# avi22bhattacharya/ThinkDiff-mlre

Hardware: AMD Instinct MI355X
Metric: images/sec (1024², 28 steps) ThinkDiff-CLIP FLUX.1 at 1/2/4/8 MI355X (higher is better)
Workload: dtype bf16

## Files before the change

### thinkdiff-mlre_amd/csrc/elementwise.hip

```cpp
#include "td_common.h"
#include "td_kernels.h"
#include "qk_rope_math.h"
#include "../../include/thinkdiff_hip.h"

namespace {

__device__ __forceinline__ void unpack8(const u32x4_t v, float (&f)[8]) {
#pragma unroll
  for (int i = 0; i < 4; ++i) {
    f[2 * i] = bf_lo(v[i]);
    f[2 * i + 1] = bf_hi(v[i]);
  }
}
__device__ __forceinline__ u32x4_t pack8(const float (&f)[8]) {
  u32x4_t v;
#pragma unroll
  for (int i = 0; i < 4; ++i) v[i] = pack_bf2(f[2 * i], f[2 * i + 1]);
  return v;
}

}

__device__ __forceinline__ u32x2_t pack8_fp8(const float (&x)[8], float inv) {
  int lo = 0, hi = 0;
  lo = __builtin_amdgcn_cvt_pk_fp8_f32(x[0] * inv, x[1] * inv, lo, false);
  lo = __builtin_amdgcn_cvt_pk_fp8_f32(x[2] * inv, x[3] * inv, lo, true);
  hi = __builtin_amdgcn_cvt_pk_fp8_f32(x[4] * inv, x[5] * inv, hi, false);
  hi = __builtin_amdgcn_cvt_pk_fp8_f32(x[6] * inv, x[7] * inv, hi, true);
  return u32x2_t{(unsigned)lo, (unsigned)hi};
}
__device__ __forceinline__ u32x2_t pack8_i8(const float (&x)[8], float inv) {
  unsigned w[2];
#pragma unroll
  for (int h = 0; h < 2; ++h) {
    const unsigned b0 = (unsigned)__float2int_rn(x[4 * h] * inv) & 0xffu, b1 = (unsigned)__float2int_rn(x[4 * h + 1] * inv) & 0xffu;
    const unsigned b2 = (unsigned)__float2int_rn(x[4 * h + 2] * inv) & 0xffu, b3 = (unsigned)__float2int_rn(x[4 * h + 3] * inv) & 0xffu;
    w[h] = b0 | (b1 << 8) | (b2 << 16) | (b3 << 24);
  }
  return u32x2_t{w[0], w[1]};
}
__device__ __forceinline__ u32x2_t pack8_q(const float (&x)[8], float inv, bool int8) { return int8 ? pack8_i8(x, inv) : pack8_fp8(x, inv); }

template <int NCH>
__global__ __launch_bounds__(256) void td_norm_rows_kernel(const TdNormParams p) {
  const int lane = threadIdx.x & 63;
  const int row = blockIdx.x * 4 + (threadIdx.x >> 6);
  if (row >= p.rows) return;
  const bf16_t* xr = p.x + (size_t)row * p.ldx;
  int ext_s0 = -1, ext_s1 = -1;
  {
    const int* ext0 = row >= p.split ? p.extB : p.extA;
    if (p.q && ext0 && lane * 2 < p.ext_n) { ext_s0 = ext0[lane * 2]; ext_s1 = ext0[lane * 2 + 1]; }
  }
  float v[NCH][8];
  float sum = 0.f;
#pragma unroll
  for (int c = 0; c < NCH; ++c) {
    unpack8(*(const u32x4_t*)(xr + c * 512 + lane * 8), v[c]);
#pragma unroll
    for (int i = 0; i < 8; ++i) sum += v[c][i];
  }
  constexpr float inv_d = 1.0f / (NCH * 512);
  float mean = 0.f;
  if (!p.rms) mean = wave_sum(sum) * inv_d;
  float sq = 0.f;
#pragma unroll
  for (int c = 0; c < NCH; ++c)
#pragma unroll
    for (int i = 0; i < 8; ++i) {
      v[c][i] -= mean;
      sq += v[c][i] * v[c][i];
    }
  const float rstd = rsqrtf(wave_sum(sq) * inv_d + p.eps);

  const bool partB = row >= p.split;
  const bf16_t* shift = partB ? p.shiftB : p.shiftA;
  const bf16_t* scale = partB ? p.scaleB : p.scaleA;
  bf16_t* yr = p.y + (size_t)row * p.ldy;
  float amax = 0.f;
#pragma unroll
  for (int c = 0; c < NCH; ++c) {
    const int col = c * 512 + lane * 8;
    float y[8];
    const bool keep_f32 = p.rms == 2;
#pragma unroll
    for (int i = 0; i < 8; ++i) y[i] = keep_f32 ? v[c][i] * rstd : rbf(v[c][i] * rstd);
    if (p.w) {
      float w[8];
      unpack8(*(const u32x4_t*)(p.w + col), w);
#pragma unroll
      for (int i = 0; i < 8; ++i) y[i] = keep_f32 ? y[i] * w[i] : rbf(y[i] * w[i]);
    }
    if (scale) {
      float sc[8], sh[8];
      unpack8(*(const u32x4_t*)(scale + col), sc);
      unpack8(*(const u32x4_t*)(shift + col), sh);
#pragma unroll
      for (int i = 0; i < 8; ++i) y[i] = rbf(rbf(y[i] * rbf(1.0f + sc[i])) + sh[i]);
    }
    if (p.q) {
      float sm[8] = {1.f, 1.f, 1.f, 1.f, 1.f, 1.f, 1.f, 1.f};
      const bf16_t* smooth = partB ? p.smoothB : p.smoothA;
      if (smooth) unpack8(*(const u32x4_t*)(smooth + col), sm);
#pragma unroll
      for (int i = 0; i < 8; ++i) {
        v[c][i] = rbf(y[i]) * sm[i];
        amax = fmaxf(amax, fabsf(v[c][i]));
      }
    } else {
      *(u32x4_t*)(yr + col) = pack8(y);
    }
  }
  if (p.q) {
    amax = wave_max(amax);
    const float s = amax > 0.f ? amax * (p.q_int8 ? 1.0f / 127.0f : 1.0f / 448.0f) : 1.0f;
    const float inv = 1.0f / s;
    if (lane == 0) p.q_scale[row] = s;
    uint8_t* qr = p.q + (size_t)row * p.ldq;
    const int* ext = partB ? p.extB : p.extA;
    __shared__ __attribute__((aligned(8))) uint8_t qrow[4][NCH * 512];
#pragma unroll
    for (int c = 0; c < NCH; ++c) {
      const u32x2_t b = pack8_q(v[c], inv, p.q_int8 != 0);
      *(u32x2_t*)(qr + c * 512 + lane * 8) = b;
      if (ext) *(u32x2_t*)(&qrow[threadIdx.x >> 6][c * 512 + lane * 8]) = b;
    }
    if (ext) {
      for (int e = lane * 2; e < p.ext_n; e += 128) {
        const int s0 = e < 128 ? ext_s0 : ext[e], s1 = e < 128 ? ext_s1 : ext[e + 1];
        const unsigned b0 = s0 >= 0 ? qrow[threadIdx.x >> 6][s0] : 0u, b1 = s1 >= 0 ? qrow[threadIdx.x >> 6][s1] : 0u;
        *(unsigned short*)(qr + NCH * 512 + e) = (unsigned short)(b0 | (b1 << 8));
      }
    }
  }
}

int td_norm_rows_launch(const TdNormParams& p, hipStream_t stream) {
  TD_CHECK_ARG(p.rows > 0 && p.D > 0, "td_norm_rows: empty problem");
  TD_CHECK_ARG(p.D % 512 == 0 && p.D <= 4096, "td_norm_rows: D=%d must be a multiple of 512, <= 4096", p.D);
  TD_CHECK_ARG(p.ldx % 8 == 0 && p.ldy % 8 == 0, "td_norm_rows: row strides must be multiples of 8");
  TD_CHECK_ARG((p.scaleA == nullptr) == (p.shiftA == nullptr), "td_norm_rows: shift and scale come together");
  if (p.q) TD_CHECK_ARG(p.q_scale && p.ldq % 8 == 0 && (uintptr_t)p.q % 8 == 0, "td_norm_rows: fp8 output needs a scale array and 8-byte aligned rows");
  if (p.extA || p.extB) TD_CHECK_ARG(p.q && p.q_int8 && p.extA && p.extB && p.ext_n > 0 && p.ext_n % 2 == 0 && p.ldq >= p.D + p.ext_n,
                                     "td_norm_rows: replicated channels need the int8 output form, both tables and rows of D + ext_n bytes");
  TD_GRID_1D(nblk, (long long)((p.rows + 3) / 4) * 256, 256, "td_norm_rows");
  const dim3 grid(nblk), block(256);
  switch (p.D / 512) {
#define TD_CASE(n) case n: hipLaunchKernelGGL(td_norm_rows_kernel<n>, grid, block, 0, stream, p); break;
    TD_CASE(1) TD_CASE(2) TD_CASE(3) TD_CASE(4) TD_CASE(5) TD_CASE(6) TD_CASE(7) TD_CASE(8)
#undef TD_CASE
  }
  TD_CHECK_LAUNCH();
  return 0;
}

__global__ __launch_bounds__(256) void td_qk_norm_rope_kernel(const TdQkRopeParams p) {
  const int row = blockIdx.x;
  const int l16 = threadIdx.x & 15;
  const int unit0 = threadIdx.x >> 4;
  const int nunits = p.Hq + p.Hk;
  bf16_t* base = p.qkv + (size_t)row * p.ld;
  const bool partB = row >= p.split;
  const bf16_t* wq = partB ? p.wqB : p.wqA;
  const bf16_t* wk = partB ? p.wkB : p.wkA;

  float cs[8], sn[8];
  {
    const float* cr = p.cos + (size_t)row * 128;
    const float* sr = p.sin + (size_t)row * 128;
    const int d0 = l16 * 8;
#pragma unroll
    for (int i = 0; i < 8; i += 4) {
      const f32x4_t c4 = *(const f32x4_t*)(cr + d0 + i);
      const f32x4_t s4 = *(const f32x4_t*)(sr + d0 + i);
#pragma unroll
      for (int j = 0; j < 4; ++j) {
        cs[i + j] = c4[j];
        sn[i + j] = s4[j];
      }
    }
  }

  for (int u = unit0; u < nunits; u += 16) {
    const bool is_k = u >= p.Hq;
    bf16_t* hp = base + (is_k ? p.k_col + (u - p.Hq) * 128 : p.q_col + u * 128) + l16 * 8;
    float x[8];
    unpack8(*(const u32x4_t*)hp, x);
    const bf16_t* w = is_k ? wk : wq;
    if (w) {
      float sq = qk_sumsq8(x);
#pragma unroll
      for (int o = 8; o > 0; o >>= 1) sq += __shfl_xor(sq, o, 16);
      float wv[8];
      unpack8(*(const u32x4_t*)(w + l16 * 8), wv);
      qk_norm8(x, qk_rstd(sq, p.eps), wv);
    }
    float y[8];
    if (p.rotate_half) {
#pragma unroll
      for (int i = 0; i < 8; ++i) {
        const float other = __shfl_xor(x[i], 8, 16);
        const float rot = (l16 < 8) ? -other : other;
        y[i] = p.rotate_half == 2 ? qk_rope_half_rbf(x[i], other, l16 < 8, cs[i], sn[i]) : x[i] * cs[i] + rot * sn[i];
      }
    } else {
      qk_rope_pairs8(x, cs, sn, y);
    }
    if (!is_k && p.q_premul != 1.0f) {
#pragma unroll
      for (int i = 0; i < 8; ++i) y[i] *= p.q_premul;
    }
    *(u32x4_t*)hp = pack8(y);
  }
}

int td_qk_norm_rope_launch(const TdQkRopeParams& p, hipStream_t stream) {
  TD_CHECK_ARG(p.rows > 0 && p.Hq > 0 && p.Hk >= 0, "td_qk_norm_rope: empty problem");
  TD_CHECK_ARG(p.ld % 8 == 0 && p.q_col % 8 == 0 && p.k_col % 8 == 0, "td_qk_norm_rope: columns must be 16-byte aligned");
  TD_CHECK_ARG(p.rotate_half >= 0 && p.rotate_half <= 2, "td_qk_norm_rope: rotate_half=%d is not a rotation mode (0, 1 or 2)", p.rotate_half);
  TD_GRID_1D(nblk, (long long)p.rows * 256, 256, "td_qk_norm_rope");
  hipLaunchKernelGGL(td_qk_norm_rope_kernel, dim3(nblk), dim3(256), 0, stream, p);
  TD_CHECK_LAUNCH();
  return 0;
}

__global__ void td_flux_rope_table_kernel(const float* ids, int S, int d0, int d1, int d2, double theta, float* cosT, float* sinT) {
  const int idx = blockIdx.x * blockDim.x + threadIdx.x;
  const int half = (d0 + d1 + d2) / 2;
  if (idx >= S * half) return;
  const int s = idx / half, j = idx % half;
  int axis, jj, dim;
  if (j < d0 / 2) { axis = 0; jj = j; dim = d0; }
  else if (j < (d0 + d1) / 2) { axis = 1; jj = j - d0 / 2; dim = d1; }
  else { axis = 2; jj = j - (d0 + d1) / 2; dim = d2; }
  const double freq = 1.0 / pow(theta, (double)(2 * jj) / (double)dim);
  const double ang = (double)ids[s * 3 + axis] * freq;
  const float c = (float)cos(ang), sn = (float)sin(ang);
  const size_t o = (size_t)s * (2 * half) + 2 * j;
  cosT[o] = c; cosT[o + 1] = c;
  sinT[o] = sn; sinT[o + 1] = sn;
}

int td_flux_rope_table_launch(const float* ids, int S, const int* axes, double theta, float* cosT, float* sinT, hipStream_t stream) {
  TD_CHECK_ARG(S > 0 && axes[0] + axes[1] + axes[2] == 128, "td_flux_rope_table: axes dims must sum to 128");
  const long long n = (long long)S * 64;
  TD_GRID_1D_I32(nblk, n, 256, "td_flux_rope_table");
  hipLaunchKernelGGL(td_flux_rope_table_kernel, dim3(nblk), dim3(256), 0, stream, ids, S, axes[0], axes[1], axes[2], theta, cosT, sinT);
  TD_CHECK_LAUNCH();
  return 0;
}

__global__ void td_timestep_sincos_kernel(const float* t, int n, bf16_t* out) {
  const int idx = blockIdx.x * blockDim.x + threadIdx.x;
  if (idx >= n * 128) return;
  const int r = idx / 128, j = idx % 128;
  const float f = expf(-9.210340371976184f * (float)j / 128.0f);
  const float a = t[r] * f;
  out[r * 256 + j] = f2bf(cosf(a));
  out[r * 256 + 128 + j] = f2bf(sinf(a));
}

int td_timestep_sincos_launch(const float* t, int n, bf16_t* out, hipStream_t stream) {
  TD_CHECK_ARG(n > 0, "td_timestep_sincos: n must be positive");
  TD_GRID_1D_I32(nblk, (long long)n * 128, 256, "td_timestep_sincos");
  hipLaunchKernelGGL(td_timestep_sincos_kernel, dim3(nblk), dim3(256), 0, stream, t, n, out);
  TD_CHECK_LAUNCH();
  return 0;
}

__global__ void td_temb_combine_silu_kernel(const bf16_t* te, const bf16_t* ge, const bf16_t* pe, int n, int D, bf16_t* temb, bf16_t* silu_out) {
  const int idx = blockIdx.x * blockDim.x + threadIdx.x;
  if (idx >= n * D) return;
  const int c = idx % D;
  float v = bf2f(te[idx]);
  if (ge) v = rbf(v + bf2f(ge[c]));
  v = rbf(v + bf2f(pe[c]));
  if (temb) temb[idx] = f2bf(v);
  silu_out[idx] = f2bf(silu_f(v));
}

int td_temb_combine_silu_launch(const bf16_t* te, const bf16_t* ge, const bf16_t* pe, int n, int D, bf16_t* temb, bf16_t* silu_out, hipStream_t stream) {
  TD_CHECK_ARG(n > 0 && D > 0, "td_temb_combine_silu: empty problem");
  TD_GRID_1D_I32(nblk, (long long)n * D, 256, "td_temb_combine_silu");
  hipLaunchKernelGGL(td_temb_combine_silu_kernel, dim3(nblk), dim3(256), 0, stream, te, ge, pe, n, D, temb, silu_out);
  TD_CHECK_LAUNCH();
  return 0;
}

__device__ __forceinline__ void euler8(float (&a)[8], const float (&b)[8], float dt) {
  const float dtb = rbf(dt);
#pragma unroll
  for (int i = 0; i < 8; ++i) a[i] = a[i] + rbf(dtb * b[i]);
}

__global__ void td_euler_step_kernel(bf16_t* x, const bf16_t* v, float dt, int n8) {
  const int idx = blockIdx.x * blockDim.x + threadIdx.x;
  if (idx >= n8) return;
  float a[8], b[8];
  unpack8(((const u32x4_t*)x)[idx], a);
  unpack8(((const u32x4_t*)v)[idx], b);
  euler8(a, b, dt);
  ((u32x4_t*)x)[idx] = pack8(a);
}

__global__ void td_flux_cfg_step_kernel(bf16_t* x, const bf16_t* vp, const bf16_t* vn, float scale, float dt, int n8) {
  const int idx = blockIdx.x * blockDim.x + threadIdx.x;
  if (idx >= n8) return;
  float a[8], p[8], q[8];
  unpack8(((const u32x4_t*)x)[idx], a);
  unpack8(((const u32x4_t*)vp)[idx], p);
  unpack8(((const u32x4_t*)vn)[idx], q);
#pragma unroll
  for (int i = 0; i < 8; ++i) p[i] = rbf(q[i] + rbf(scale * rbf(p[i] - q[i])));
  euler8(a, p, dt);
  ((u32x4_t*)x)[idx] = pack8(a);
}

int td_flux_cfg_step_launch(bf16_t* x, const bf16_t* v_pos, const bf16_t* v_neg, float scale, float dt, long long n, hipStream_t stream) {
  TD_CHECK_ARG(x && v_pos && v_neg, "td_flux_cfg_step: null argument");
  TD_CHECK_ARG(n > 0 && n % 8 == 0, "td_flux_cfg_step: n=%lld must be a positive multiple of 8", n);
  TD_CHECK_ARG(((uintptr_t)x | (uintptr_t)v_pos | (uintptr_t)v_neg) % 16 == 0, "td_flux_cfg_step: every buffer must be 16-byte aligned");
  const uintptr_t x0 = (uintptr_t)x, x1 = x0 + (uintptr_t)n * sizeof(bf16_t);
  for (const bf16_t* o : {v_pos, v_neg})
    TD_CHECK_ARG((uintptr_t)o >= x1 || (uintptr_t)o + (uintptr_t)n * sizeof(bf16_t) <= x0,
                 "td_flux_cfg_step: v_pos and v_neg must not overlap x (updated in place)");
  TD_GRID_1D_I32(nblk, n / 8, 256, "td_flux_cfg_step");
  hipLaunchKernelGGL(td_flux_cfg_step_kernel, dim3(nblk), dim3(256), 0, stream, x, v_pos, v_neg, scale, dt, (int)(n / 8));
  TD_CHECK_LAUNCH();
  return 0;
}

__global__ void td_flux_inpaint_step_kernel(bf16_t* x, const bf16_t* v, const bf16_t* z, const bf16_t* noise, const bf16_t* mask,
                                            float dt, float sigma_next, int n8) {
  const int idx = blockIdx.x * blockDim.x + threadIdx.x;
  if (idx >= n8) return;
  float a[8], b[8], p[8], m[8];
  unpack8(((const u32x4_t*)x)[idx], a);
  unpack8(((const u32x4_t*)v)[idx], b);
  unpack8(((const u32x4_t*)z)[idx], p);
  unpack8(((const u32x4_t*)mask)[idx], m);
  euler8(a, b, dt);
  if (noise) {
    float e[8];
    unpack8(((const u32x4_t*)noise)[idx], e);
    const float s = rbf(sigma_next), oms = rbf(1.0f - s);
#pragma unroll
    for (int i = 0; i < 8; ++i) p[i] = rbf(rbf(s * e[i]) + rbf(oms * p[i]));
  }
#pragma unroll
  for (int i = 0; i < 8; ++i) a[i] = rbf(rbf(1.0f - m[i]) * p[i]) + rbf(m[i] * rbf(a[i]));
  ((u32x4_t*)x)[idx] = pack8(a);
}

int td_flux_inpaint_step_launch(bf16_t* x, const bf16_t* v, const bf16_t* z, const bf16_t* noise, const bf16_t* mask, float dt,
                                float sigma_next, long long n, hipStream_t stream) {
  TD_CHECK_ARG(x && v && z && mask, "td_flux_inpaint_step: null argument (x, v, image_latents and mask are required)");
  TD_CHECK_ARG(n > 0 && n % 8 == 0, "td_flux_inpaint_step: n=%lld must be a positive multiple of 8", n);
  TD_CHECK_ARG(((uintptr_t)x | (uintptr_t)v | (uintptr_t)z | (uintptr_t)noise | (uintptr_t)mask) % 16 == 0,
               "td_flux_inpaint_step: every buffer must be 16-byte aligned");
  const uintptr_t x0 = (uintptr_t)x, x1 = x0 + (uintptr_t)n * sizeof(bf16_t);
  for (const bf16_t* o : {z, noise, mask})
    TD_CHECK_ARG(!o || (uintptr_t)o >= x1 || (uintptr_t)o + (uintptr_t)n * sizeof(bf16_t) <= x0,
                 "td_flux_inpaint_step: image_latents, noise and mask must not overlap x (updated in place)");
  TD_GRID_1D_I32(nblk, n / 8, 256, "td_flux_inpaint_step");
  hipLaunchKernelGGL(td_flux_inpaint_step_kernel, dim3(nblk), dim3(256), 0, stream, x, v, z, noise, mask, dt, sigma_next, (int)(n / 8));
  TD_CHECK_LAUNCH();
  return 0;
}

__global__ void td_flux_inpaint_mask_kernel(const void* src, int fmt, int H, int W, int C, bf16_t* out) {
  const int chunks = C >> 1, w2 = W >> 4;
  const int idx = blockIdx.x * blockDim.x + threadIdx.x;
  if (idx >= (H >> 4) * w2 * chunks) return;
  const int tok = idx / chunks;
  const int ty = tok / w2, tx = tok - ty * w2;
  float q[4];
#pragma unroll
  for (int k = 0; k < 4; ++k) {
    const size_t pix = (size_t)(16 * ty + 8 * (k >> 1)) * W + 16 * tx + 8 * (k & 1);
    const bool on = fmt == TD_INPAINT_MASK_U8_HW ? ((const unsigned char*)src)[pix] >= 128 : ((const float*)src)[pix] >= 0.5f;
    q[k] = on ? 1.0f : 0.0f;
  }
  const unsigned lo = pack_bf2(q[0], q[1]), hi = pack_bf2(q[2], q[3]);
  *(u32x4_t*)(out + (size_t)idx * 8) = u32x4_t{lo, hi, lo, hi};
}

int td_flux_inpaint_mask_launch(const void* mask, int fmt, int H, int W, int C, bf16_t* out, hipStream_t stream) {
  TD_CHECK_ARG(mask && out, "td_flux_inpaint_mask: null argument");
  TD_CHECK_ARG(fmt == TD_INPAINT_MASK_U8_HW || fmt == TD_INPAINT_MASK_F32_HW, "td_flux_inpaint_mask: unknown mask format %d", fmt);
  TD_CHECK_ARG(H > 0 && W > 0 && H % 16 == 0 && W % 16 == 0, "td_flux_inpaint_mask: H=%d, W=%d must be positive multiples of 16", H, W);
  TD_CHECK_ARG(C > 0 && C % 2 == 0, "td_flux_inpaint_mask: C=%d must be a positive multiple of 2 (4C columns in 8-column chunks)", C);
  TD_CHECK_ARG(((uintptr_t)out) % 16 == 0, "td_flux_inpaint_mask: packed_out must be 16-byte aligned");
  TD_GRID_1D_I32(nblk, (long long)(H / 16) * (W / 16) * (C / 2), 256, "td_flux_inpaint_mask");
  hipLaunchKernelGGL(td_flux_inpaint_mask_kernel, dim3(nblk), dim3(256), 0, stream, mask, fmt, H, W, C, out);
  TD_CHECK_LAUNCH();
  return 0;
}

__global__ void td_copy_cols_kernel(const bf16_t* src, int lds, bf16_t* dst, int ldd, int rows, int chunks) {
  const int idx = blockIdx.x * blockDim.x + threadIdx.x;
  if (idx >= rows * chunks) return;
  const int r = idx / chunks, c = idx - r * chunks;
  *(u32x4_t*)(dst + (size_t)r * ldd + c * 8) = *(const u32x4_t*)(src + (size_t)r * lds + c * 8);
}

int td_copy_cols_launch(const bf16_t* src, int lds, bf16_t* dst, int ldd, int rows, int cols, hipStream_t stream) {
  TD_CHECK_ARG(src && dst && rows > 0 && cols > 0, "td_copy_cols: empty problem");
  TD_CHECK_ARG(cols % 8 == 0 && lds % 8 == 0 && ldd % 8 == 0 && cols <= lds && cols <= ldd, "td_copy_cols: cols=%d, lds=%d, ldd=%d must be multiples of 8, cols within both", cols, lds, ldd);
  TD_CHECK_ARG(((uintptr_t)src | (uintptr_t)dst) % 16 == 0, "td_copy_cols: both buffers must be 16-byte aligned");
  TD_GRID_1D_I32(nblk, (long long)rows * (cols / 8), 256, "td_copy_cols");
  hipLaunchKernelGGL(td_copy_cols_kernel, dim3(nblk), dim3(256), 0, stream, src, lds, dst, ldd, rows, cols / 8);
  TD_CHECK_LAUNCH();
  return 0;
}

__global__ void td_flux_residual_inject_kernel(bf16_t* h, int ldh, const bf16_t* r, int ldr, int rows, int chunks, float scale) {
  const int idx = blockIdx.x * blockDim.x + threadIdx.x;
  if (idx >= rows * chunks) return;
  const int m = idx / chunks, c = idx - m * chunks;
  bf16_t* hp = h + (size_t)m * ldh + c * 8;
  float a[8], b[8];
  unpack8(*(const u32x4_t*)hp, a);
  unpack8(*(const u32x4_t*)(r + (size_t)m * ldr + c * 8), b);
#pragma unroll
  for (int i = 0; i < 8; ++i) a[i] = a[i] + rbf(scale * b[i]);
  *(u32x4_t*)hp = pack8(a);
}

int td_flux_residual_inject_launch(bf16_t* h, int ldh, const bf16_t* r, int ldr, int rows, int D, float scale, hipStream_t stream) {
  TD_CHECK_ARG(h && r, "td_flux_residual_inject: null argument");
  TD_CHECK_ARG(rows > 0 && D > 0 && D % 8 == 0, "td_flux_residual_inject: rows=%d, D=%d: D must be a positive multiple of 8, rows positive", rows, D);
  TD_CHECK_ARG(ldh % 8 == 0 && ldr % 8 == 0 && ldh >= D && ldr >= D, "td_flux_residual_inject: ldh=%d, ldr=%d must be multiples of 8 and at least D=%d", ldh, ldr, D);
  TD_CHECK_ARG(((uintptr_t)h | (uintptr_t)r) % 16 == 0, "td_flux_residual_inject: both buffers must be 16-byte aligned");
  const uintptr_t h0 = (uintptr_t)h, h1 = h0 + ((uintptr_t)(rows - 1) * ldh + D) * sizeof(bf16_t);
  const uintptr_t r0 = (uintptr_t)r, r1 = r0 + ((uintptr_t)(rows - 1) * ldr + D) * sizeof(bf16_t);
  TD_CHECK_ARG(r0 >= h1 || r1 <= h0, "td_flux_residual_inject: r must not overlap h (updated in place)");
  TD_GRID_1D_I32(nblk, (long long)rows * (D / 8), 256, "td_flux_residual_inject");
  hipLaunchKernelGGL(td_flux_residual_inject_kernel, dim3(nblk), dim3(256), 0, stream, h, ldh, r, ldr, rows, D / 8, scale);
  TD_CHECK_LAUNCH();
  return 0;
}

struct TdInjectMultiArgs {
  const bf16_t* r[TD_MAX_CONTROLNETS];
  int ldr[TD_MAX_CONTROLNETS];
  float scale[TD_MAX_CONTROLNETS];
};

template <int N>
__global__ void td_flux_residual_inject_multi_kernel(bf16_t* h, int ldh, TdInjectMultiArgs p, int rows, int chunks) {
  const int idx = blockIdx.x * blockDim.x + threadIdx.x;
  if (idx >= rows * chunks) return;
  const int m = idx / chunks, c = idx - m * chunks;
  bf16_t* hp = h + (size_t)m * ldh + c * 8;
  float a[8], acc[8], b[8];
  unpack8(*(const u32x4_t*)hp, a);
  unpack8(*(const u32x4_t*)(p.r[0] + (size_t)m * p.ldr[0] + c * 8), b);
#pragma unroll
  for (int i = 0; i < 8; ++i) acc[i] = rbf(p.scale[0] * b[i]);
#pragma unroll
  for (int k = 1; k < N; ++k) {
    unpack8(*(const u32x4_t*)(p.r[k] + (size_t)m * p.ldr[k] + c * 8), b);
#pragma unroll
    for (int i = 0; i < 8; ++i) acc[i] = rbf(acc[i] + rbf(p.scale[k] * b[i]));
  }
#pragma unroll
  for (int i = 0; i < 8; ++i) a[i] = a[i] + acc[i];
  *(u32x4_t*)hp = pack8(a);
}

int td_flux_residual_inject_multi_launch(bf16_t* h, int ldh, const bf16_t* const* r, const int* ldr, const float* scales, int n, int rows, int D,
                                         hipStream_t stream) {
  TD_CHECK_ARG(h && r && ldr && scales, "td_flux_residual_inject_multi: null argument");
  TD_CHECK_ARG(n >= 1 && n <= TD_MAX_CONTROLNETS, "td_flux_residual_inject_multi: n=%d outside 1 .. %d", n, TD_MAX_CONTROLNETS);
  TD_CHECK_ARG(rows > 0 && D > 0 && D % 8 == 0, "td_flux_residual_inject_multi: rows=%d, D=%d: D must be a positive multiple of 8, rows positive", rows, D);
  TD_CHECK_ARG(ldh % 8 == 0 && ldh >= D, "td_flux_residual_inject_multi: ldh=%d must be a multiple of 8 and at least D=%d", ldh, D);
  TD_CHECK_ARG((uintptr_t)h % 16 == 0, "td_flux_residual_inject_multi: h must be 16-byte aligned");
  const uintptr_t h0 = (uintptr_t)h, h1 = h0 + ((uintptr_t)(rows - 1) * ldh + D) * sizeof(bf16_t);
  TdInjectMultiArgs p = {};
  for (int k = 0; k < n; ++k) {
    TD_CHECK_ARG(r[k], "td_flux_residual_inject_multi: r[%d] is null", k);
    TD_CHECK_ARG(ldr[k] % 8 == 0 && ldr[k] >= D, "td_flux_residual_inject_multi: ldr[%d]=%d must be a multiple of 8 and at least D=%d", k, ldr[k], D);
    TD_CHECK_ARG((uintptr_t)r[k] % 16 == 0, "td_flux_residual_inject_multi: r[%d] must be 16-byte aligned", k);
    TD_CHECK_ARG(std::isfinite(scales[k]), "td_flux_residual_inject_multi: scales[%d] is not finite", k);
    const uintptr_t r0 = (uintptr_t)r[k], r1 = r0 + ((uintptr_t)(rows - 1) * ldr[k] + D) * sizeof(bf16_t);
    TD_CHECK_ARG(r0 >= h1 || r1 <= h0, "td_flux_residual_inject_multi: r[%d] must not overlap h (updated in place)", k);
    p.r[k] = r[k]; p.ldr[k] = ldr[k]; p.scale[k] = scales[k];
  }
  TD_GRID_1D_I32(nblk, (long long)rows * (D / 8), 256, "td_flux_residual_inject_multi");
  const dim3 grid(nblk), block(256);
  switch (n) {
    case 1: hipLaunchKernelGGL(td_flux_residual_inject_multi_kernel<1>, grid, block, 0, stream, h, ldh, p, rows, D / 8); break;
    case 2: hipLaunchKernelGGL(td_flux_residual_inject_multi_kernel<2>, grid, block, 0, stream, h, ldh, p, rows, D / 8); break;
    case 3: hipLaunchKernelGGL(td_flux_residual_inject_multi_kernel<3>, grid, block, 0, stream, h, ldh, p, rows, D / 8); break;
    default: hipLaunchKernelGGL(td_flux_residual_inject_multi_kernel<4>, grid, block, 0, stream, h, ldh, p, rows, D / 8); break;
  }
  TD_CHECK_LAUNCH();
  return 0;
}

int td_euler_step_launch(bf16_t* x, const bf16_t* v, float dt, long long n, hipStream_t stream) {
  TD_CHECK_ARG(n > 0 && n % 8 == 0, "td_euler_step: n=%lld must be a positive multiple of 8", n);
  TD_GRID_1D_I32(nblk, n / 8, 256, "td_euler_step");
  const int n8 = (int)(n / 8);
  hipLaunchKernelGGL(td_euler_step_kernel, dim3(nblk), dim3(256), 0, stream, x, v, dt, n8);
  TD_CHECK_LAUNCH();
  return 0;
}

__global__ void td_flux_pack_kernel(const bf16_t* src, bf16_t* dst, int C, int H, int W, int unpack, float div, float add) {
  const int idx = blockIdx.x * blockDim.x + threadIdx.x;
  const int total = C * H * W;
  if (idx >= total) return;
  const int cols = C * 4;
  const int tok = idx / cols, col = idx % cols;
  const int c = col >> 2, di = (col >> 1) & 1, dj = col & 1;
  const int wj = W / 2;
  const int i = tok / wj, j = tok % wj;
  const size_t sp = ((size_t)c * H + (2 * i + di)) * W + (2 * j + dj);
  if (unpack) dst[sp] = f2bf(__fadd_rn(rbf(__fdiv_rn(bf2f(src[idx]), div)), rbf(add)));
// ... 469 lines not shown
```

### thinkdiff-mlre_amd/csrc/td_common.h

```cpp
#pragma once
#include <hip/hip_runtime.h>
#include <stdint.h>

typedef uint16_t bf16_t;

typedef __attribute__((ext_vector_type(8))) short bf16x8_t;
typedef __attribute__((ext_vector_type(4))) short bf16x4_t;
typedef __attribute__((ext_vector_type(4))) float f32x4_t;
typedef __attribute__((ext_vector_type(16))) float f32x16_t;
typedef __attribute__((ext_vector_type(4))) unsigned u32x4_t;
typedef __attribute__((ext_vector_type(2))) unsigned u32x2_t;
typedef __attribute__((ext_vector_type(2))) __bf16 bf16x2_t;

#define TD_LDS __attribute__((address_space(3)))

__device__ __forceinline__ float bf2f(bf16_t v) {
  return __builtin_bit_cast(float, (unsigned)v << 16);
}
__device__ __forceinline__ bf16_t f2bf(float f) {
  return __builtin_bit_cast(bf16_t, (__bf16)f);
}
__device__ __forceinline__ unsigned pack_bf2(float lo, float hi) {
  typedef __attribute__((ext_vector_type(2))) __bf16 v2;
  v2 p;
  p[0] = (__bf16)lo;
  p[1] = (__bf16)hi;
  return __builtin_bit_cast(unsigned, p);
}
__device__ __forceinline__ unsigned as_u32(float f) { return __builtin_bit_cast(unsigned, f); }
__device__ __forceinline__ float as_f32(unsigned u) { return __builtin_bit_cast(float, u); }
__device__ __forceinline__ float rbf(float f) { return bf2f(f2bf(f)); }
__device__ __forceinline__ float bf_lo(unsigned u) { return __builtin_bit_cast(float, u << 16); }
__device__ __forceinline__ float bf_hi(unsigned u) { return __builtin_bit_cast(float, u & 0xffff0000u); }
__device__ __forceinline__ float dot8(const u32x4_t& a, const u32x4_t& b, float acc) {
#pragma unroll
  for (int q = 0; q < 4; ++q) {
    const unsigned ua = a[q], ub = b[q];
    acc = __builtin_amdgcn_fdot2_f32_bf16(__builtin_bit_cast(bf16x2_t, ua), __builtin_bit_cast(bf16x2_t, ub), acc, false);
  }
  return acc;
}

__device__ __forceinline__ float sigmoid_f(float z) {
  return __builtin_amdgcn_rcpf(1.0f + __builtin_amdgcn_exp2f(-1.4426950408889634f * z));
}
__device__ __forceinline__ float gelu_tanh_f(float x) {
  return x * sigmoid_f(x * (1.5957691216057308f + 0.07135481627260025f * x * x));
}
__device__ __forceinline__ float gelu_erf_f(float x) {
  return 0.5f * x * (1.0f + erff(x * 0.7071067811865476f));
}
__device__ __forceinline__ float silu_f(float x) { return x * sigmoid_f(x); }
__device__ __forceinline__ float quick_gelu_f(float x) { return x * sigmoid_f(1.702f * x); }

__device__ __forceinline__ float wave_sum(float v) {
#pragma unroll
  for (int o = 32; o > 0; o >>= 1) v += __shfl_xor(v, o, 64);
  return v;
}
__device__ __forceinline__ float wave_max(float v) {
#pragma unroll
  for (int o = 32; o > 0; o >>= 1) v = fmaxf(v, __shfl_xor(v, o, 64));
  return v;
}

__device__ __forceinline__ float row16_xor8(float v) {
  return __builtin_bit_cast(float, __builtin_amdgcn_update_dpp(0, __builtin_bit_cast(int, v), 0x128, 0xf, 0xf, false));
}
__device__ __forceinline__ float row16_sum(float s) {
  s += row16_xor8(s);
  s += __builtin_bit_cast(float, __builtin_amdgcn_update_dpp(0, __builtin_bit_cast(int, s), 0x124, 0xf, 0xf, false));
  s += __builtin_bit_cast(float, __builtin_amdgcn_update_dpp(0, __builtin_bit_cast(int, s), 0x122, 0xf, 0xf, false));
  s += __builtin_bit_cast(float, __builtin_amdgcn_update_dpp(0, __builtin_bit_cast(int, s), 0x121, 0xf, 0xf, false));
  return s;
}
__device__ __forceinline__ float row16_max(float s) {
  s = fmaxf(s, row16_xor8(s));
  s = fmaxf(s, __builtin_bit_cast(float, __builtin_amdgcn_update_dpp(0, __builtin_bit_cast(int, s), 0x124, 0xf, 0xf, false)));
  s = fmaxf(s, __builtin_bit_cast(float, __builtin_amdgcn_update_dpp(0, __builtin_bit_cast(int, s), 0x122, 0xf, 0xf, false)));
  s = fmaxf(s, __builtin_bit_cast(float, __builtin_amdgcn_update_dpp(0, __builtin_bit_cast(int, s), 0x121, 0xf, 0xf, false)));
  return s;
}

void td_set_error(const char* fmt, ...);
#define TD_CHECK_ARG(cond, ...)          \
  do {                                   \
    if (!(cond)) {                       \
      td_set_error(__VA_ARGS__);         \
      return 2;      \
    }                                    \
  } while (0)
#define TD_CHECK_HIP(expr)                                                        \
  do {                                                                            \
    hipError_t _e = (expr);                                                       \
    if (_e != hipSuccess) {                                                       \
      td_set_error("%s failed: %s (%s:%d)", #expr, hipGetErrorString(_e), __FILE__, __LINE__); \
      return 3;                                                   \
    }                                                                             \
  } while (0)
#define TD_CHECK_LAUNCH() TD_CHECK_HIP(hipGetLastError())
#define TD_TRY(expr)          \
  do {                        \
    int _rc = (expr);         \
    if (_rc != 0) return _rc; \
  } while (0)

inline bool td_grid_1d(long long items, int block, unsigned* blocks) {
  if (items <= 0 || block <= 0) return false;
  const long long b = (items + block - 1) / block;
  if (b * block >= (1ll << 32)) return false;
  *blocks = (unsigned)b;
  return true;
}
#define TD_GRID_1D(var, items, block, what)                                                                                   \
  unsigned var = 0;                                                                                                           \
  TD_CHECK_ARG(td_grid_1d((long long)(items), (block), &var),                                                                 \
               "%s: %lld work-items in blocks of %d do not fit one launch (grid x block must stay below 2^32)", what, (long long)(items), (int)(block))
#define TD_GRID_1D_I32(var, items, block, what)                                                                               \
  TD_CHECK_ARG((long long)(items) < (1ll << 31), "%s: %lld work-items exceed the kernel's 32-bit index", what, (long long)(items)); \
  TD_GRID_1D(var, items, block, what)
```

Baseline: 0.6318.

## Specialize non-quantized row norm kernel with templated weight/modulation and DPP wave reductions

Splits the row normalization into a quantized path and a new non-quantized kernel templated on whether a weight and shift/scale modulation are present. The new kernel keeps the input as packed bf16 registers and re-unpacks it, using empty asm barriers so the compiler does not hold a float copy live. It loads modulation eagerly when registers allow, sets waves-per-EU hints, and swaps the shuffle-based wave sum for permlane-swap plus DPP reductions. The aim is lower register pressure and cheaper reductions in a memory-bound kernel, at the cost of inline asm that is tied to the gfx950 target and of more template instances.

Measured after the change: 0.6318, median of 4. Within noise of the previous version (+0.0%).

```diff
diff --git a/thinkdiff-mlre_amd/csrc/elementwise.hip b/thinkdiff-mlre_amd/csrc/elementwise.hip
--- a/thinkdiff-mlre_amd/csrc/elementwise.hip
+++ b/thinkdiff-mlre_amd/csrc/elementwise.hip
@@ -19,6 +19,14 @@
   return v;
 }
 
+__device__ __forceinline__ void repack_barrier(u32x4_t& v) {
+#pragma unroll
+  for (int i = 0; i < 4; ++i) {
+    unsigned t = v[i];
+    asm volatile("" : "+v"(t));
+    v[i] = t;
+  }
+}
 }
 
 __device__ __forceinline__ u32x2_t pack8_fp8(const float (&x)[8], float inv) {
@@ -41,8 +49,85 @@
 }
 __device__ __forceinline__ u32x2_t pack8_q(const float (&x)[8], float inv, bool int8) { return int8 ? pack8_i8(x, inv) : pack8_fp8(x, inv); }
 
+template <int NCH, bool HAS_W, bool MOD>
+__global__ __launch_bounds__(256) __attribute__((amdgpu_waves_per_eu(NCH <= 6 && !HAS_W ? 5 : (NCH <= 4 ? 4 : 2)))) void td_norm_rows_kernel(const TdNormParams p) {
+#pragma clang fp contract(off)
+  constexpr bool EAGER_MOD = MOD && !HAS_W && NCH <= 6;
+  const int lane = threadIdx.x & 63;
+  const int row = blockIdx.x * 4 + (threadIdx.x >> 6);
+  if (row >= p.rows) return;
+  const bf16_t* xr = p.x + (size_t)row * p.ldx;
+  const bool partB = row >= p.split;
+  const bf16_t* shift = partB ? p.shiftB : p.shiftA;
+  const bf16_t* scale = partB ? p.scaleB : p.scaleA;
+  u32x4_t xv[NCH], wv[HAS_W ? NCH : 1], sc[EAGER_MOD ? NCH : 1], sh[EAGER_MOD ? NCH : 1];
+#pragma unroll
+  for (int c = 0; c < NCH; ++c) xv[c] = *(const u32x4_t*)(xr + c * 512 + lane * 8);
+  if (HAS_W) {
+#pragma unroll
+    for (int c = 0; c < NCH; ++c) wv[c] = *(const u32x4_t*)(p.w + c * 512 + lane * 8);
+  }
+  if (EAGER_MOD) {
+#pragma unroll
+    for (int c = 0; c < NCH; ++c) {
+      sc[c] = *(const u32x4_t*)(scale + c * 512 + lane * 8);
+      sh[c] = *(const u32x4_t*)(shift + c * 512 + lane * 8);
+    }
+  }
+  float sum = 0.f;
+#pragma unroll
+  for (int c = 0; c < NCH; ++c)
+#pragma unroll
+    for (int i = 0; i < 4; ++i) {
+      sum += bf_lo(xv[c][i]);
+      sum += bf_hi(xv[c][i]);
+    }
+  constexpr float inv_d = 1.0f / (NCH * 512);
+  float mean = 0.f;
+  if (!p.rms) mean = wave_sum_dpp(sum) * inv_d;
+  float sq = 0.f;
+#pragma unroll
+  for (int c = 0; c < NCH; ++c) repack_barrier(xv[c]);
+#pragma unroll
+  for (int c = 0; c < NCH; ++c)
+#pragma unroll
+    for (int i = 0; i < 4; ++i) {
+      const float d0 = bf_lo(xv[c][i]) - mean, d1 = bf_hi(xv[c][i]) - mean;
+      sq += d0 * d0;
+      sq += d1 * d1;
+    }
+  const float rstd = rsqrtf(__builtin_fmaf(wave_sum_dpp(sq), inv_d, p.eps));
+#pragma unroll
+  for (int c = 0; c < NCH; ++c) repack_barrier(xv[c]);
+
+  bf16_t* yr = p.y + (size_t)row * p.ldy;
+  const bool keep_f32 = p.rms == 2;
+#pragma unroll
+  for (int c = 0; c < NCH; ++c) {
+    const int col = c * 512 + lane * 8;
+    float x[8], y[8];
+    unpack8(xv[c], x);
+#pragma unroll
+    for (int i = 0; i < 8; ++i) y[i] = keep_f32 ? (x[i] - mean) * rstd : rbf((x[i] - mean) * rstd);
+    if (HAS_W) {
+      float w[8];
+      unpack8(wv[c], w);
+#pragma unroll
+      for (int i = 0; i < 8; ++i) y[i] = keep_f32 ? y[i] * w[i] : rbf(y[i] * w[i]);
+    }
+    if (MOD) {
+      float s1[8], s0[8];
+      unpack8(EAGER_MOD ? sc[c] : *(const u32x4_t*)(scale + col), s1);
+      unpack8(EAGER_MOD ? sh[c] : *(const u32x4_t*)(shift + col), s0);
+#pragma unroll
+      for (int i = 0; i < 8; ++i) y[i] = rbf(rbf(y[i] * rbf(1.0f + s1[i])) + s0[i]);
+    }
+    *(u32x4_t*)(yr + col) = pack8(y);
+  }
+}
+
 template <int NCH>
-__global__ __launch_bounds__(256) void td_norm_rows_kernel(const TdNormParams p) {
+__global__ __launch_bounds__(256) void td_norm_rows_quant_kernel(const TdNormParams p) {
   const int lane = threadIdx.x & 63;
   const int row = blockIdx.x * 4 + (threadIdx.x >> 6);
   if (row >= p.rows) return;
@@ -145,10 +230,20 @@
                                      "td_norm_rows: replicated channels need the int8 output form, both tables and rows of D + ext_n bytes");
   TD_GRID_1D(nblk, (long long)((p.rows + 3) / 4) * 256, 256, "td_norm_rows");
   const dim3 grid(nblk), block(256);
+  const bool mod = p.scaleA != nullptr;
   switch (p.D / 512) {
-#define TD_CASE(n) case n: hipLaunchKernelGGL(td_norm_rows_kernel<n>, grid, block, 0, stream, p); break;
+#define TD_LAUNCH(...) hipLaunchKernelGGL((__VA_ARGS__), grid, block, 0, stream, p)
+#define TD_CASE(n)                                                        \
+  case n:                                                                 \
+    if (p.q) TD_LAUNCH(td_norm_rows_quant_kernel<n>);                     \
+    else if (p.w && mod) TD_LAUNCH(td_norm_rows_kernel<n, true, true>);   \
+    else if (p.w) TD_LAUNCH(td_norm_rows_kernel<n, true, false>);         \
+    else if (mod) TD_LAUNCH(td_norm_rows_kernel<n, false, true>);         \
+    else TD_LAUNCH(td_norm_rows_kernel<n, false, false>);                 \
+    break;
     TD_CASE(1) TD_CASE(2) TD_CASE(3) TD_CASE(4) TD_CASE(5) TD_CASE(6) TD_CASE(7) TD_CASE(8)
 #undef TD_CASE
+#undef TD_LAUNCH
   }
   TD_CHECK_LAUNCH();
   return 0;
@@ -215,7 +310,7 @@
 }
 
 int td_qk_norm_rope_launch(const TdQkRopeParams& p, hipStream_t stream) {
-  TD_CHECK_ARG(p.rows > 0 && p.Hq > 0 && p.Hk >= 0, "td_qk_norm_rope: empty problem");
+  TD_CHECK_ARG(p.rows > 0 && p.Hq >= 0 && p.Hk >= 0 && p.Hq + p.Hk > 0, "td_qk_norm_rope: empty problem");
   TD_CHECK_ARG(p.ld % 8 == 0 && p.q_col % 8 == 0 && p.k_col % 8 == 0, "td_qk_norm_rope: columns must be 16-byte aligned");
   TD_CHECK_ARG(p.rotate_half >= 0 && p.rotate_half <= 2, "td_qk_norm_rope: rotate_half=%d is not a rotation mode (0, 1 or 2)", p.rotate_half);
   TD_GRID_1D(nblk, (long long)p.rows * 256, 256, "td_qk_norm_rope");
diff --git a/thinkdiff-mlre_amd/csrc/td_common.h b/thinkdiff-mlre_amd/csrc/td_common.h
--- a/thinkdiff-mlre_amd/csrc/td_common.h
+++ b/thinkdiff-mlre_amd/csrc/td_common.h
@@ -82,6 +82,16 @@
   return s;
 }
 
+__device__ __forceinline__ float wave_sum_dpp(float v) {
+  float a = v, b = v;
+  asm volatile("s_nop 1\n\tv_permlane32_swap_b32 %0, %1\n\ts_nop 1" : "+v"(a), "+v"(b));
+  v = a + b;
+  a = v;
+  b = v;
+  asm volatile("s_nop 1\n\tv_permlane16_swap_b32 %0, %1\n\ts_nop 1" : "+v"(a), "+v"(b));
+  return row16_sum(a + b);
+}
+
 void td_set_error(const char* fmt, ...);
 #define TD_CHECK_ARG(cond, ...)          \
   do {                                   \
```
